# bluecube/minipath

Hardware: AMD Instinct MI355X
Metric: Mrays/s (higher is better)
Workload: dtype f32; 1 GPU; atrium stand-in for the absent data/Sponza (reference .gitmodules:1-3: un-fetched submodule), 258432 triangles, generator seed 1; 1920x1080 256spp tile64 seed0x5eed depth1 (reference semantics: primary ray + |d.n|, worker.rs:51-66); parallelism=tiles round-robin over 1 rank(s)

## Files before the change

### minipath_amd/csrc/kernels.hip

```cpp
#include <hip/hip_runtime.h>

#include <algorithm>
#include <cfloat>
#include <cmath>
#include <cstdlib>
#include <type_traits>

#include "launch_plan.h"
#include "mp_internal.h"
#include "family_launch.h"
#include "ray_math.h"

#ifdef MP_PROF_MISSES
namespace mp {
namespace {
__device__ unsigned long long g_prof[8];
}
}
#define MP_PROF_COUNT(i) do { if ((threadIdx.x & 63u) == 0u) atomicAdd(&g_prof[i], 1ull); } while (0)
#endif
#include "mask_cache.h"
#include "group_walk.h"

namespace mp {
// ... 327 lines not shown
                const float hx = fms(r.dy, e2z, r.dz * e2y), hy = fms(r.dz, e2x, r.dx * e2z), hz = fms(r.dx, e2y, r.dy * e2x);
                const float det = fma_dot(e1x, e1y, e1z, hx, hy, hz);
                const float sx = r.ox - v0x, sy = r.oy - v0y, sz = r.oz - v0z;
                const float un = fma_dot(sx, sy, sz, hx, hy, hz);
                const uint32_t det_sign = as_u(det) & 0x80000000u;
                const bool det_ok = fabsf(det) <= kHuge;
                const float xu = det_ok ? as_f(as_u(un) ^ det_sign) : 1.0f;
                if (__ballot(!(xu <= thr)) == 0) return;
                const float qx = fms(sy, e1z, sz * e1y), qy = fms(sz, e1x, sx * e1z), qz = fms(sx, e1y, sy * e1x);
                const float vn = fma_dot(r.dx, r.dy, r.dz, qx, qy, qz);
                const float tn = fma_dot(e2x, e2y, e2z, qx, qy, qz);
                const float xv = det_ok ? as_f(as_u(vn) ^ det_sign) : 1.0f, xt = det_ok ? as_f(as_u(tn) ^ det_sign) : 1.0f;
                if (__ballot(!(fminf(fminf(xu, xv), xt) <= thr)) == 0) return;
                const float inv_det = 1.0f / det;
                const float u = inv_det * un, v = inv_det * vn, t = inv_det * tn;
                const bool acc = (u >= 0.0f) & (v >= 0.0f) & ((u + v) <= 1.0f) & (t >= 0.0f) & (t < lim);
                best_t = acc ? t : best_t;
                lim = acc ? t : lim;
                bu = acc ? u : bu;
                bv = acc ? v : bv;
                bprim = acc ? tri : bprim;
                changed |= __ballot(acc);
            };
            float a0 = tp[0], a1 = tp[1], a2 = tp[2], a3 = tp[3], a4 = tp[4], a5 = tp[5], a6 = tp[6], a7 = tp[7], a8 = tp[8];
            uint32_t tri = first * 8u;
            for (uint32_t p = n_real >> 1; p > 0; p--) {
                const float b0 = tp[9], b1 = tp[10], b2 = tp[11], b3 = tp[12], b4 = tp[13], b5 = tp[14], b6 = tp[15], b7 = tp[16], b8 = tp[17];
                test(a0, a1, a2, a3, a4, a5, a6, a7, a8, tri);
                a0 = tp[18]; a1 = tp[19]; a2 = tp[20]; a3 = tp[21]; a4 = tp[22]; a5 = tp[23]; a6 = tp[24]; a7 = tp[25]; a8 = tp[26];
                test(b0, b1, b2, b3, b4, b5, b6, b7, b8, tri + 1u);
                tri += 2u;
                tp += 2 * kTriDwords;
            }
            if (n_real & 1u) test(a0, a1, a2, a3, a4, a5, a6, a7, a8, tri);
            if (changed != 0) stale_top = sp;
        }
    }
    hit.t = best_t; hit.u = bu; hit.v = bv; hit.prim = bprim;
}

struct RegStack3 {
    int ent, mlo, mhi;
    __device__ __forceinline__ RegStack3() : ent(0), mlo(0), mhi(0) {}
    __device__ __forceinline__ void push(int sp, uint32_t e, uint64_t m) {
        asm volatile("s_mov_b32 m0, %3\n\ts_nop 0\n\t"
                     "v_writelane_b32 %0, %4, m0\n\tv_writelane_b32 %1, %5, m0\n\tv_writelane_b32 %2, %6, m0"
                     : "+v"(ent), "+v"(mlo), "+v"(mhi)
                     : "s"(sp), "s"(e), "s"(static_cast<uint32_t>(m)), "s"(static_cast<uint32_t>(m >> 32))
                     : "m0");
    }
    __device__ __forceinline__ void pop(int sp, uint32_t& e, uint64_t& m) const {
        e = static_cast<uint32_t>(__builtin_amdgcn_readlane(ent, sp));
        m = static_cast<uint32_t>(__builtin_amdgcn_readlane(mlo, sp)) |
            (static_cast<uint64_t>(static_cast<uint32_t>(__builtin_amdgcn_readlane(mhi, sp))) << 32);
    }
};

template <int OCT>
__device__ __noinline__ uint32_t unit_list_slow(const float* __restrict__ nodes_pk, uint32_t* mcache, uint32_t node, uint32_t slots) {
    return unit_list_build(reinterpret_cast<const float4*>(nodes_pk), mcache, node, slots,
                           [](const float* b, const float bmn[3], const float bmx[3]) { return bounds_may_hit<OCT>(b, bmn, bmx); });
}
template <int OCT>
__device__ __forceinline__ bool trace_packet_cached(const DevScene& sc, const Ray& r, bool active, PacketHit& hit, uint32_t* mcache) {
    static_assert(kNullLink == MP_LINK_NULL, "mask_cache.h's copy of the null link");
    kfp nodes = (kfp)(uintptr_t)sc.nodes_pk;
    kfp tris = (kfp)(uintptr_t)sc.tris_aos;
    float best_t = FLT_MAX, bu = 0.0f, bv = 0.0f;
    uint32_t bprim = kNoPrim;
    RegStack3 st;
    int sp = 0;
    mcache[kRootListSlot] = sc.pk_count * sc.pk_mask_bits;
    wave_lds_sync();
    uint32_t cur = (static_cast<uint32_t>(kRootListSlot) << 16) | 1u;
    uint64_t pm = __ballot(active);
    for (;;) {
        if ((cur & 0xFFFFu) == 0u) {
            if (sp == 0) break;
            sp--;
            st.pop(sp, cur, pm);
        }
        cur -= 1u;
        const uint32_t src = __builtin_amdgcn_readfirstlane(mcache[(cur >> 16) + (cur & 0xFFFFu)]);
        const bool pon = __builtin_amdgcn_inverse_ballot_w64(pm);
        const krec8 rec = *reinterpret_cast<const __attribute__((address_space(4))) krec8*>(reinterpret_cast<const __attribute__((address_space(4))) char*>(nodes) + scalar_u(src * 32u));
        float t1, t2;
        slab<false, OCT>(rec[0], rec[1], rec[2], rec[3], rec[4], rec[5], r, pon ? best_t : -1.0f, t1, t2);
        const bool ok = t1 <= t2;
        if (__ballot(ok) == 0) continue;
        const uint32_t link = uniform_u(rec[6]);
        float lim = ok ? best_t : -1.0f;
        if ((link & 63u) == 0u) {
            MP_PROF_COUNT(2);
            const uint32_t node = link >> 6;
            const uint32_t slot = node_slot(node);
            const uint32_t tag = __builtin_amdgcn_readfirstlane(mcache[static_cast<uint32_t>(kMaskCacheHeader) + slot]);
            uint32_t list = __builtin_amdgcn_readfirstlane(mcache[static_cast<uint32_t>(kNodeListBase) + slot]);
            if (__builtin_expect(tag != node, 0)) {
                MP_PROF_COUNT(0);
                if (tag != 0xFFFFFFFFu) MP_PROF_COUNT(4);
                list = __builtin_amdgcn_readfirstlane(unit_list_slow<OCT>(sc.nodes_pk, mcache, node, sc.pk_mask_bits));
                if (list == kListOverflow) {
                    if (sp != 0 || (cur & 0xFFFFu) != 0u) {
                        MP_PROF_COUNT(6);
                        return false;
                    }
                    list = __builtin_amdgcn_readfirstlane(unit_list_slow<OCT>(sc.nodes_pk, mcache, node, sc.pk_mask_bits));
                }
            }
            if ((list & 0xFFFFu) != 0u) {
                if ((cur & 0xFFFFu) != 0u) {
                    st.push(sp, cur, pm);
                    sp++;
                }
                cur = list;
                pm = __ballot(lim >= 0.0f);
            }
        } else {
            const uint32_t first = link >> 6, n_real = link & 63u;
            kfp tp = tris + static_cast<size_t>(first) * (8 * kTriDwords);
            const float thr = lim >= 0.0f ? -kTiny : INFINITY;
            auto test = [&](const float v0x, const float v0y, const float v0z, const float e1x, const float e1y, const float e1z,
                            const float e2x, const float e2y, const float e2z, const uint32_t tri) {
                const float hx = fms(r.dy, e2z, r.dz * e2y), hy = fms(r.dz, e2x, r.dx * e2z), hz = fms(r.dx, e2y, r.dy * e2x);
                const float det = fma_dot(e1x, e1y, e1z, hx, hy, hz);
                const float sx = r.ox - v0x, sy = r.oy - v0y, sz = r.oz - v0z;
                const float un = fma_dot(sx, sy, sz, hx, hy, hz);
                const uint32_t det_sign = as_u(det) & 0x80000000u;
                const bool det_ok = fabsf(det) <= kHuge;
                const float xu = det_ok ? as_f(as_u(un) ^ det_sign) : 1.0f;
                if (__ballot(!(xu <= thr)) == 0) return;
                const float qx = fms(sy, e1z, sz * e1y), qy = fms(sz, e1x, sx * e1z), qz = fms(sx, e1y, sy * e1x);
                const float vn = fma_dot(r.dx, r.dy, r.dz, qx, qy, qz);
                const float tn = fma_dot(e2x, e2y, e2z, qx, qy, qz);
                const float xv = det_ok ? as_f(as_u(vn) ^ det_sign) : 1.0f, xt = det_ok ? as_f(as_u(tn) ^ det_sign) : 1.0f;
                if (__ballot(!(fminf(fminf(xu, xv), xt) <= thr)) == 0) return;
                constexpr uint32_t kRcpLo = 0x10800000u , kRcpHi = 0x7E000000u ;
                const uint32_t wkey = (as_u(det) << 1) - (kRcpLo << 1);
                const float inv_det = __ballot(wkey > ((kRcpHi - kRcpLo) << 1)) == 0 ? rm::rcp_short(det) : 1.0f / det;
                const float u = inv_det * un, v = inv_det * vn, t = inv_det * tn;
                const bool acc = !(fminf(fminf(u, v), t) < 0.0f) & ((u + v) <= 1.0f) & (t < lim);
                best_t = acc ? t : best_t;
                lim = acc ? t : lim;
                bu = acc ? u : bu;
                bv = acc ? v : bv;
                bprim = acc ? tri : bprim;
            };
            const uint32_t ls = first & static_cast<uint32_t>(kLeafCacheEntries - 1);
            const uint32_t tag = mcache[kLeafTagBase + ls];
            const uint2 tm = reinterpret_cast<const uint2*>(mcache + kLeafMaskBase)[ls];
            uint64_t todo;
            if (__builtin_expect(__builtin_amdgcn_readfirstlane(tag) == first, 1)) {
                todo = __builtin_amdgcn_readfirstlane(tm.x) | (static_cast<uint64_t>(__builtin_amdgcn_readfirstlane(tm.y)) << 32);
            } else {
                MP_PROF_COUNT(1);
                const uint64_t m = leaf_mask_slow(sc.tris_aos, mcache, first, n_real);
                todo = __builtin_amdgcn_readfirstlane(static_cast<uint32_t>(m)) | (static_cast<uint64_t>(__builtin_amdgcn_readfirstlane(static_cast<uint32_t>(m >> 32))) << 32);
            }
            if (todo != 0) {
                uint32_t c = static_cast<uint32_t>(__builtin_ctzll(todo));
                todo &= ~(1ull << c);
                kfp ta = tri_record(tp, c);
                krec8 ra = *reinterpret_cast<const __attribute__((address_space(4))) krec8*>(ta);
                float a8 = ta[8];
                while (todo != 0) {
                    const uint32_t cn = static_cast<uint32_t>(__builtin_ctzll(todo));
                    todo &= ~(1ull << cn);
                    kfp tb = tri_record(tp, cn);
                    const krec8 rb = *reinterpret_cast<const __attribute__((address_space(4))) krec8*>(tb);
                    const float b8 = tb[8];
                    test(ra[0], ra[1], ra[2], ra[3], ra[4], ra[5], ra[6], ra[7], a8, first * 8u + c);
                    ra = rb; a8 = b8;
                    c = cn;
                }
                test(ra[0], ra[1], ra[2], ra[3], ra[4], ra[5], ra[6], ra[7], a8, first * 8u + c);
            }
        }
    }
    hit.t = best_t; hit.u = bu; hit.v = bv; hit.prim = bprim;
    return true;
}

template <bool OCTANTS, class Stack, bool MC = false>
__device__ __forceinline__ void trace_packet(const DevScene& sc, const Ray& r, bool active, Stack& st, PacketHit& hit,
                                             const MaskCache& mc = MaskCache{nullptr}) {
    if (OCTANTS && MC) {
        if (__ballot(active & !mask_cache_ray_ok(r)) != 0) {
            const bool slow = active && (fabsf(r.ix) == INFINITY || fabsf(r.iy) == INFINITY || fabsf(r.iz) == INFINITY);
            if (__ballot(slow) != 0) trace_packet_impl<2, -1>(sc, r, active, st, hit);
            else trace_packet_impl<1, -1>(sc, r, active, st, hit);
            return;
        }
    } else {
        const bool slow = active && (fabsf(r.ix) == INFINITY || fabsf(r.iy) == INFINITY || fabsf(r.iz) == INFINITY);
        if (__ballot(slow) != 0) {
            trace_packet_impl<2, -1>(sc, r, active, st, hit);
            return;
        }
    }
    if (OCTANTS && sc.boxes_ordered) {
        const uint64_t am = __ballot(active);
        const uint64_t nx = __ballot(active && r.ix < 0.0f), ny = __ballot(active && r.iy < 0.0f), nz = __ballot(active && r.iz < 0.0f);
        if ((nx == 0 || nx == am) && (ny == 0 || ny == am) && (nz == 0 || nz == am)) {
            const uint32_t oct = (nx ? 1u : 0u) | (ny ? 2u : 0u) | (nz ? 4u : 0u);
            if (MC) {
                mask_cache_begin_pass(mc, r, active, oct);
                bool done;
                switch (oct) {
                    case 0: done = trace_packet_cached<0>(sc, r, active, hit, mc.lds); break;
                    case 1: done = trace_packet_cached<1>(sc, r, active, hit, mc.lds); break;
                    case 2: done = trace_packet_cached<2>(sc, r, active, hit, mc.lds); break;
                    case 3: done = trace_packet_cached<3>(sc, r, active, hit, mc.lds); break;
                    case 4: done = trace_packet_cached<4>(sc, r, active, hit, mc.lds); break;
                    case 5: done = trace_packet_cached<5>(sc, r, active, hit, mc.lds); break;
                    case 6: done = trace_packet_cached<6>(sc, r, active, hit, mc.lds); break;
                    default: done = trace_packet_cached<7>(sc, r, active, hit, mc.lds); break;
                }
                if (done) return;
            } else {
                switch (oct) {
                    case 0: trace_packet_impl<1, 0>(sc, r, active, st, hit); return;
                    case 1: trace_packet_impl<1, 1>(sc, r, active, st, hit); return;
                    case 2: trace_packet_impl<1, 2>(sc, r, active, st, hit); return;
                    case 3: trace_packet_impl<1, 3>(sc, r, active, st, hit); return;
                    case 4: trace_packet_impl<1, 4>(sc, r, active, st, hit); return;
                    case 5: trace_packet_impl<1, 5>(sc, r, active, st, hit); return;
                    case 6: trace_packet_impl<1, 6>(sc, r, active, st, hit); return;
                    default: trace_packet_impl<1, 7>(sc, r, active, st, hit); return;
                }
            }
        }
    }
    trace_packet_impl<1, -1>(sc, r, active, st, hit);
}

template <class T>
__device__ __forceinline__ const T* uniform_ptr(const T* p) {
    const uint64_t v = reinterpret_cast<uint64_t>(p);
    const uint32_t lo = __builtin_amdgcn_readfirstlane(static_cast<uint32_t>(v)), hi = __builtin_amdgcn_readfirstlane(static_cast<uint32_t>(v >> 32));
    return reinterpret_cast<const T*>((static_cast<uint64_t>(hi) << 32) | lo);
}
// ... 1549 lines not shown
```

### minipath_amd/csrc/mask_cache.h

```cpp
#pragma once

#include <hip/hip_runtime.h>

#include <cfloat>
#include <cmath>
#include <cstdint>

#include "camera_rays.h"

#ifndef MP_PROF_COUNT
#define MP_PROF_COUNT(i) do { } while (0)
#endif

namespace mp {
namespace mc {
__device__ __forceinline__ float as_f(uint32_t u) { return __uint_as_float(u); }
__device__ __forceinline__ uint32_t as_u(float f) { return __float_as_uint(f); }

__device__ __forceinline__ void wave_lds_sync() {
    __builtin_amdgcn_fence(__ATOMIC_RELEASE, "wavefront");
    __builtin_amdgcn_wave_barrier();
    __builtin_amdgcn_fence(__ATOMIC_ACQUIRE, "wavefront");
}

// ... 148 lines not shown
            for (int g = 0; g < 3; g++) {
#pragma unroll
                for (int k = 0; k < 3; k++) { hdr[hdr_lo(g) + k] = pmin[g][k]; hdr[hdr_lo(g) + 3 + k] = pmax[g][k]; }
            }
            mc.lds[kHdrState] = oct | 0x100u;
        }
        int l_ = lane;
        asm volatile("" : "+v"(l_));
#pragma unroll
        for (int i = 0; i < (kMaskCacheEntries + kLeafCacheEntries) / 64; i++) mc.lds[kMaskCacheHeader + i * 64 + l_] = 0xFFFFFFFFu;
        wave_lds_sync();
    }
}
#ifndef MP_MCACHE_MARGIN
#define MP_MCACHE_MARGIN 0.015625f
#endif
__device__ __forceinline__ void mask_cache_begin_unit(const MaskCache& mc, const mp_camera_sampler& s, float jitter_scale, uint32_t x0,
                                                      uint32_t x1, uint32_t y0, uint32_t y1) {
    const int lane = static_cast<int>(threadIdx.x) & 63;
    Ray r;
    float f[3];
    camera_film(s, (lane & 1) ? static_cast<float>(x1) + (jitter_scale + (-0.5f)) : static_cast<float>(x0) + (-0.5f),
                (lane & 2) ? static_cast<float>(y1) + (jitter_scale + (-0.5f)) : static_cast<float>(y0) + (-0.5f), f);
    camera_lens_ray(s, f, (lane & 4) ? 1.0f : -1.0f, (lane & 8) ? 1.0f : -1.0f, r);
    const uint64_t nx = __ballot(r.ix < 0.0f), ny = __ballot(r.iy < 0.0f), nz = __ballot(r.iz < 0.0f);
    const bool adopt = __ballot(!mask_cache_ray_ok(r)) == 0 && (nx == 0 || ~nx == 0) && (ny == 0 || ~ny == 0) && (nz == 0 || ~nz == 0);
    if (!adopt) {
        if (lane == 0) mc.lds[kHdrState] = 0xFFFFFFFFu;
        wave_lds_sync();
        return;
    }
    const uint32_t oct = (nx ? 1u : 0u) | (ny ? 2u : 0u) | (nz ? 4u : 0u);
    float pmin[3][3] = {{r.ox, r.oy, r.oz}, {r.ix, r.iy, r.iz}, {r.dx, r.dy, r.dz}}, pmax[3][3];
#pragma unroll
    for (int g = 0; g < 3; g++) {
#pragma unroll
        for (int k = 0; k < 3; k++) pmax[g][k] = pmin[g][k];
        wave_min3_max3(pmin[g], pmax[g]);
    }
    float* hdr = reinterpret_cast<float*>(mc.lds);
    if (lane == 63) {
#pragma unroll
        for (int g = 0; g < 3; g++) {
#pragma unroll
            for (int k = 0; k < 3; k++) {
                const float lo = pmin[g][k], hi = pmax[g][k];
                const float pad = (hi - lo) * MP_MCACHE_MARGIN;
                float wlo = lo - pad, whi = hi + pad;
                if (g == 1) {
                    if ((wlo < 0.0f) != (lo < 0.0f) || wlo == 0.0f) wlo = lo;
                    if ((whi < 0.0f) != (hi < 0.0f) || whi == 0.0f) whi = hi;
                    if (!(fabsf(wlo) < INFINITY)) wlo = lo;
                    if (!(fabsf(whi) < INFINITY)) whi = hi;
                } else {
                    const float cap = g == 0 ? 2.0f * kCoordCap : 2.0f;
                    wlo = fmaxf(wlo, -cap); whi = fminf(whi, cap);
                }
                hdr[hdr_lo(g) + k] = wlo; hdr[hdr_lo(g) + 3 + k] = whi;
            }
        }
        mc.lds[kHdrState] = oct | 0x100u;
    }
    MP_PROF_COUNT(3);
#pragma unroll
    for (int i = 0; i < (kMaskCacheEntries + kLeafCacheEntries) / 64; i++) mc.lds[kMaskCacheHeader + i * 64 + lane] = 0xFFFFFFFFu;
    wave_lds_sync();
}
template <int OCT>
__device__ __forceinline__ bool bounds_may_hit(const float* b, const float bmn[3], const float bmx[3]) {
    float L[3], U[3];
#pragma unroll
    for (int k = 0; k < 3; k++) {
        const float y = bmn[k] - b[3 + k], z = bmx[k] - b[k];
        const float lo_src = ((OCT >> k) & 1) ? z : y, hi_src = ((OCT >> k) & 1) ? y : z;
        L[k] = fminf(lo_src * b[6 + k], lo_src * b[9 + k]);
        U[k] = fmaxf(hi_src * b[6 + k], hi_src * b[9 + k]);
    }
    const float t1 = fmaxf(fmaxf(L[0], 0.0f), fmaxf(L[1], L[2])), t2 = fminf(U[0], fminf(U[1], U[2]));
    return !(t1 > t2);
}

constexpr uint32_t kNullLink = 0xFFFFFFF8u;
constexpr uint32_t kListOverflow = 0xFFFFFFFFu;
constexpr int kListDepth = 64;
__device__ __forceinline__ uint32_t node_slot(uint32_t node) {
    return min(node & static_cast<uint32_t>(kMaskCacheEntries - 1) & MP_NODE_SLOT_MASK, static_cast<uint32_t>(kMaskCacheEntries - 2));
}
template <class Kept>
__device__ __forceinline__ uint32_t unit_list_build(const float4* __restrict__ recs, uint32_t* mcache, uint32_t node, uint32_t slots, Kept kept) {
    const uint32_t lane = threadIdx.x & 63u;
    const float* b = reinterpret_cast<const float*>(mcache);
    node = __builtin_amdgcn_readfirstlane(node);
    slots = __builtin_amdgcn_readfirstlane(slots);
    auto kept_of = [&](uint32_t n, float4& c0, float4& c1) -> uint32_t {
        bool keep = false;
        c0 = make_float4(0.0f, 0.0f, 0.0f, 0.0f); c1 = c0;
        if (lane < slots) {
            const float4* r = recs + (static_cast<size_t>(n) * slots + lane) * 2;
            c0 = r[0]; c1 = r[1];
            const float bmn[3] = {c0.x, c0.y, c0.z}, bmx[3] = {c0.w, c1.x, c1.y};
            keep = as_u(c1.z) != kNullLink && kept(b, bmn, bmx);
        }
        return __builtin_amdgcn_readfirstlane(static_cast<uint32_t>(__ballot(keep)));
    };
    float4 c0, c1;
    uint32_t mask = kept_of(node, c0, c1);
    const uint32_t top = ~__builtin_amdgcn_readfirstlane(mcache[kArenaTopSlot]);
    if (top > static_cast<uint32_t>(kArenaEntries) || top + static_cast<uint32_t>(__popc(mask)) > static_cast<uint32_t>(kArenaEntries)) {
        MP_PROF_COUNT(5);
        wave_lds_sync();
#pragma unroll
        for (int i = 0; i < (kMaskCacheEntries + 63) / 64; i++)
            if (i * 64 + static_cast<int>(lane) < kMaskCacheEntries) mcache[kMaskCacheHeader + i * 64 + static_cast<int>(lane)] = 0xFFFFFFFFu;
        wave_lds_sync();
        return kListOverflow;
    }
    const uint32_t room = static_cast<uint32_t>(kArenaEntries) - top;
    uint32_t used = 0u, pend = static_cast<uint32_t>(__popc(mask)), cur = node;
    int st_node = 0, st_mask = 0, depth = 0;
    for (;;) {
        if (mask == 0u) {
            while (mask == 0u && depth > 0) {
                depth--;
                cur = static_cast<uint32_t>(__builtin_amdgcn_readlane(st_node, depth));
                mask = static_cast<uint32_t>(__builtin_amdgcn_readlane(st_mask, depth));
            }
            if (mask == 0u) break;
            if (lane < slots) {
                const float4* r = recs + (static_cast<size_t>(cur) * slots + lane) * 2;
                c0 = r[0]; c1 = r[1];
            }
        }
        const uint32_t j = static_cast<uint32_t>(__builtin_ctz(mask));
        mask &= mask - 1u;
        pend--;
        const uint32_t rec = cur * slots + j;
        auto from_lane = [&](float v) { return as_f(static_cast<uint32_t>(__builtin_amdgcn_readlane(static_cast<int>(as_u(v)), static_cast<int>(j)))); };
        const float4 p0 = make_float4(from_lane(c0.x), from_lane(c0.y), from_lane(c0.z), from_lane(c0.w));
        const float4 p1 = make_float4(from_lane(c1.x), from_lane(c1.y), from_lane(c1.z), 0.0f);
        const uint32_t link = as_u(p1.z);
        bool emit = true;
        if ((link & 63u) == 0u) {
            const uint32_t m = link >> 6;
            float4 g0, g1;
            const uint32_t km = kept_of(m, g0, g1);
            const bool sticks_out = ((km >> lane) & 1u) != 0u && lane < slots &&
                                    !(p0.x <= g0.x && p0.y <= g0.y && p0.z <= g0.z && g0.w <= p0.w && g1.x <= p1.x && g1.y <= p1.y);
            if (km == 0u) {
                emit = false;
            } else if (__ballot(sticks_out) == 0 && depth < kListDepth && used + pend + static_cast<uint32_t>(__popc(km)) <= room) {
                if (mask != 0u) {
                    asm volatile("s_mov_b32 m0, %2\n\ts_nop 0\n\tv_writelane_b32 %0, %3, m0\n\tv_writelane_b32 %1, %4, m0"
                                 : "+v"(st_node), "+v"(st_mask) : "s"(depth), "s"(__builtin_amdgcn_readfirstlane(cur)), "s"(__builtin_amdgcn_readfirstlane(mask)) : "m0");
                    depth++;
                }
                cur = m; mask = km; pend += static_cast<uint32_t>(__popc(km));
                c0 = g0; c1 = g1;
                emit = false;
            }
        }
        if (emit) {
            if (lane == 0u) mcache[static_cast<uint32_t>(kArenaBase) + top + used] = rec;
            used++;
        }
    }
    const uint32_t val = ((static_cast<uint32_t>(kArenaBase) + top) << 16) | used;
    if (lane == 0u) {
        const uint32_t slot = node_slot(node);
        mcache[static_cast<uint32_t>(kMaskCacheHeader) + slot] = node;
        mcache[static_cast<uint32_t>(kNodeListBase) + slot] = val;
        mcache[kArenaTopSlot] = ~(top + used);
    }
    wave_lds_sync();
    return val;
}

struct Iv {
    float lo, hi;
};
__device__ __forceinline__ Iv iv_neg(const Iv a) { return Iv{-a.hi, -a.lo}; }
__device__ __forceinline__ Iv iv_mul_c(const Iv a, const float c) {
    const float p = a.lo * c, q = a.hi * c;
    return Iv{fminf(p, q), fmaxf(p, q)};
}
__device__ __forceinline__ Iv iv_mul(const Iv a, const Iv b) {
    const float p1 = a.lo * b.lo, p2 = a.lo * b.hi, p3 = a.hi * b.lo, p4 = a.hi * b.hi;
    return Iv{fminf(fminf(p1, p2), fminf(p3, p4)), fmaxf(fmaxf(p1, p2), fmaxf(p3, p4))};
}
__device__ __forceinline__ Iv iv_fma_c(const Iv a, const float c, const Iv z) {
    return Iv{fminf(__builtin_fmaf(a.lo, c, z.lo), __builtin_fmaf(a.hi, c, z.lo)), fmaxf(__builtin_fmaf(a.lo, c, z.hi), __builtin_fmaf(a.hi, c, z.hi))};
}
__device__ __forceinline__ Iv iv_fma(const Iv a, const Iv b, const Iv z) {
    const float l1 = __builtin_fmaf(a.lo, b.lo, z.lo), l2 = __builtin_fmaf(a.lo, b.hi, z.lo), l3 = __builtin_fmaf(a.hi, b.lo, z.lo), l4 = __builtin_fmaf(a.hi, b.hi, z.lo);
    const float h1 = __builtin_fmaf(a.lo, b.lo, z.hi), h2 = __builtin_fmaf(a.lo, b.hi, z.hi), h3 = __builtin_fmaf(a.hi, b.lo, z.hi), h4 = __builtin_fmaf(a.hi, b.hi, z.hi);
    return Iv{fminf(fminf(l1, l2), fminf(l3, l4)), fmaxf(fmaxf(h1, h2), fmaxf(h3, h4))};
}
__device__ __forceinline__ bool tri_may_hit(const float* b, const float (&v0)[3], const float (&e1)[3], const float (&e2)[3]) {
    const Iv d[3] = {Iv{b[13], b[16]}, Iv{b[14], b[17]}, Iv{b[15], b[18]}};
    const Iv h[3] = {iv_fma_c(d[1], e2[2], iv_neg(iv_mul_c(d[2], e2[1]))), iv_fma_c(d[2], e2[0], iv_neg(iv_mul_c(d[0], e2[2]))),
                     iv_fma_c(d[0], e2[1], iv_neg(iv_mul_c(d[1], e2[0])))};
    const Iv det = iv_fma_c(h[2], e1[2], iv_fma_c(h[1], e1[1], iv_mul_c(h[0], e1[0])));
    if (!(det.lo > 0.0f || det.hi < 0.0f)) return true;
    const Iv inv = Iv{1.0f / det.hi, 1.0f / det.lo};
    if (!(fabsf(inv.lo) < INFINITY && fabsf(inv.hi) < INFINITY)) return true;
    const Iv s[3] = {Iv{b[0] - v0[0], b[3] - v0[0]}, Iv{b[1] - v0[1], b[4] - v0[1]}, Iv{b[2] - v0[2], b[5] - v0[2]}};
    const Iv u = iv_mul(inv, iv_fma(s[2], h[2], iv_fma(s[1], h[1], iv_mul(s[0], h[0]))));
    const Iv q[3] = {iv_fma_c(s[1], e1[2], iv_neg(iv_mul_c(s[2], e1[1]))), iv_fma_c(s[2], e1[0], iv_neg(iv_mul_c(s[0], e1[2]))),
                     iv_fma_c(s[0], e1[1], iv_neg(iv_mul_c(s[1], e1[0])))};
    const Iv v = iv_mul(inv, iv_fma(d[2], q[2], iv_fma(d[1], q[1], iv_mul(d[0], q[0]))));
    const Iv t = iv_mul(inv, iv_fma_c(q[2], e2[2], iv_fma_c(q[1], e2[1], iv_mul_c(q[0], e2[0]))));
    const bool miss = u.hi < 0.0f || v.hi < 0.0f || (u.lo + v.lo) > 1.0f || t.hi < 0.0f;
    return !miss;
}

}
}
```

### minipath_amd/csrc/mask_probe.hip

```cpp
#include <hip/hip_runtime.h>

#include <cfloat>
#include <cstdint>

#include "mask_cache.h"

namespace {

using namespace mp::mc;

constexpr int kCounters = 8;
constexpr float kOrgCap = 2.0f * kCoordCap;

__device__ __forceinline__ uint64_t mix64(uint64_t z) {
    z = (z ^ (z >> 30)) * 0xbf58476d1ce4e5b9ull;
    z = (z ^ (z >> 27)) * 0x94d049bb133111ebull;
    return z ^ (z >> 31);
}
__device__ __forceinline__ uint64_t hsh(uint64_t seed, uint64_t c, uint32_t k) { return mix64(seed ^ mix64(c * 0x10000ull + k)); }
__device__ __forceinline__ float unit(uint64_t h) { return static_cast<float>(static_cast<uint32_t>(h >> 40)) * 0x1p-24f; }

__device__ __forceinline__ void record_case(unsigned long long* out, bool bad, uint64_t idx, bool hit, bool rejected, bool edge_only) {
    if ((threadIdx.x & 63) != 0) return;
    atomicAdd(out + 1, 1ull);
// ... 121 lines not shown
        if (mode == 2u) {
            const uint64_t hn = hsh(seed, c, 42);
            const uint32_t n = 1u + static_cast<uint32_t>(hn & 3u), kk = static_cast<uint32_t>(hn >> 8) % 3u, which = static_cast<uint32_t>(hn >> 16) & 3u;
            const bool up = (hn >> 24) & 1u;
            for (uint32_t i = 0; i < n; i++) {
#pragma unroll
                for (int k = 0; k < 3; k++) {
                    if (static_cast<uint32_t>(k) != kk) continue;
                    if (which == 0u || which == 3u) v0[k] = step(v0[k], up);
                    if (which == 1u || which == 3u) v1[k] = step(v1[k], up);
                    if (which == 2u || which == 3u) v2[k] = step(v2[k], up);
                }
            }
        }
    } else if (mode == 3u) {
        const uint32_t sub = static_cast<uint32_t>(hm >> 20) & 3u, ax = static_cast<uint32_t>(hm >> 24) % 3u;
#pragma unroll
        for (int k = 0; k < 3; k++) {
            v0[k] = p[k];
            if (sub == 0u) { v1[k] = k == static_cast<int>(ax) ? p[k] + E1[k] : p[k]; v2[k] = k == static_cast<int>(ax) ? p[k] - E2[k] : p[k]; }
            else if (sub == 1u) { v1[k] = p[k]; v2[k] = p[k] + E2[k]; }
            else if (sub == 2u) { v1[k] = p[k] + E1[k]; v2[k] = v1[k]; }
            else { v1[k] = p[k] + E1[k]; v2[k] = p[k] + 2.0f * E1[k]; }
        }
    } else if (mode == 4u) {
        const uint32_t ax = static_cast<uint32_t>(hm >> 20) % 3u;
        const float f = clampf((hm >> 24) & 1u ? b[3 + ax] : b[ax], -kCoordCap, kCoordCap);
        const float a = unit(hsh(seed, c, 40)), bb = unit(hsh(seed, c, 41)) * (1.0f - a);
#pragma unroll
        for (int k = 0; k < 3; k++) {
            v0[k] = p[k] - a * E1[k] - bb * E2[k];
            v1[k] = v0[k] + E1[k];
            v2[k] = v0[k] + E2[k];
            if (k == static_cast<int>(ax)) v0[k] = v1[k] = v2[k] = f;
        }
    } else {
#pragma unroll
        for (int k = 0; k < 3; k++) {
            const float ctr = 0.5f * b[k] + 0.5f * b[3 + k];
            v0[k] = ctr + pick(hsh(seed, c, 50 + k), 127 - 30, 127 + 30);
            v1[k] = ctr + pick(hsh(seed, c, 53 + k), 127 - 30, 127 + 30);
            v2[k] = ctr + pick(hsh(seed, c, 56 + k), 127 - 30, 127 + 30);
        }
    }
    clamp_vertex(v0); clamp_vertex(v1); clamp_vertex(v2);
}

constexpr int kDumpHead = 40, kDumpRay = 10, kRays = 192;
constexpr int kDumpCase = kDumpHead + kRays * kDumpRay;

__global__ void tri_kernel(uint64_t seed, uint64_t base, uint64_t ncases, unsigned long long* out, uint32_t* dump) {
    const uint64_t c = base + (static_cast<uint64_t>(blockIdx.x) * blockDim.x + threadIdx.x) / 64u;
    const uint32_t lane = threadIdx.x & 63u;
    if (c >= ncases) return;
    float b[20], v0[3], v1[3], v2[3];
    gen_tri_case(seed, c, b, v0, v1, v2);
    const float e1[3] = {v1[0] - v0[0], v1[1] - v0[1], v1[2] - v0[2]}, e2[3] = {v2[0] - v0[0], v2[1] - v0[1], v2[2] - v0[2]};
    float lo[6], hi[6];
#pragma unroll
    for (int k = 0; k < 3; k++) { lo[k] = b[k]; hi[k] = b[3 + k]; lo[3 + k] = b[13 + k]; hi[3 + k] = b[16 + k]; }
    const bool keep = tri_may_hit(b, v0, e1, e2);
    bool edge = false, inner = false;
    uint32_t* rec = dump ? dump + c * kDumpCase : nullptr;
    for (uint32_t s = 0; s < 3; s++) {
        const uint32_t j = s * 64u + lane;
        float x[6];
        case_ray(lo, hi, j, seed, c, x);
        const TriRay tr = mt_ray(x, v0, e1, e2);
        if (s < 2) edge |= tr.hit; else inner |= tr.hit;
        if (rec) {
            uint32_t* rr = rec + kDumpHead + j * kDumpRay;
            for (int k = 0; k < 6; k++) rr[k] = as_u(x[k]);
            rr[6] = as_u(tr.t); rr[7] = as_u(tr.u); rr[8] = as_u(tr.v); rr[9] = tr.hit ? 1u : 0u;
        }
    }
    const bool any_edge = __ballot(edge) != 0, any_inner = __ballot(inner) != 0, any = any_edge || any_inner;
    if (rec && lane < 20u) rec[lane] = as_u(b[lane]);
    if (rec && lane == 20u) {
        for (int k = 0; k < 3; k++) { rec[20 + k] = as_u(v0[k]); rec[23 + k] = as_u(v1[k]); rec[26 + k] = as_u(v2[k]); }
        for (int k = 0; k < 3; k++) { rec[29 + k] = as_u(e1[k]); rec[32 + k] = as_u(e2[k]); }
        rec[35] = keep ? 1u : 0u;
    }
    record_case(out, !keep && any, c, any, !keep, any_edge && !any_inner);
}

__device__ __forceinline__ void gen_box_case(uint64_t seed, uint64_t c, uint32_t oct, float (&b)[20], float (&bmn)[3], float (&bmx)[3]) {
    float olo[3], ohi[3];
    gen_origin_bounds(seed, c, olo, ohi);
#pragma unroll
    for (int k = 0; k < 3; k++) {
        const uint64_t h = hsh(seed, c, 60 + k), h2 = hsh(seed, c, 63 + k);
        const bool wide = (h & 0x300u) == 0u;
        float m1 = wide ? pick_pos(h, 1, 254) : pick_pos(h, 127 - 2, 127 + 12);
        float m2 = (h2 & 7u) == 0u ? m1 : wide ? pick_pos(h2, 1, 254) : pick_pos(h2, 127 - 2, 127 + 12);
        if ((h2 & 0x7F00u) == 0u) m2 = FLT_MAX;
        const float mlo = fminf(m1, m2), mhi = fmaxf(m1, m2);
        const bool neg = ((oct >> k) & 1u) != 0u;
        b[k] = olo[k]; b[3 + k] = ohi[k];
        b[6 + k] = neg ? -mhi : mlo;
        b[9 + k] = neg ? -mlo : mhi;
    }
    b[12] = as_f(oct | 0x100u);
    for (int i = 13; i < 20; i++) b[i] = 0.0f;
    float lo[6], hi[6];
#pragma unroll
    for (int k = 0; k < 3; k++) { lo[k] = b[k]; hi[k] = b[3 + k]; lo[3 + k] = b[6 + k]; hi[3 + k] = b[9 + k]; }
    const uint64_t hm = hsh(seed, c, 70);
    const uint32_t mode = static_cast<uint32_t>(hm & 7u);
    float x[6];
    const uint32_t j = (hm & 0x300u) ? static_cast<uint32_t>(hm >> 10) & 127u : 128u + (static_cast<uint32_t>(hm >> 10) & 63u);
    case_ray(lo, hi, j, seed, c, x);
    const float d[3] = {1.0f / x[3], 1.0f / x[4], 1.0f / x[5]};
    const uint64_t ht = hsh(seed, c, 71);
    const float t = mode == 2u ? -pick_pos(ht, 127 - 10, 127 + 30) : (ht & 3u) == 0u ? 0.0f : pick_pos(ht, 127 - 30, 127 + 30);
    float half[3];
#pragma unroll
    for (int k = 0; k < 3; k++) {
        const float p = x[k] + t * d[k];
        half[k] = pick_pos(hsh(seed, c, 72 + k), 127 - 30, 127 + 31);
        bmn[k] = p - half[k];
        bmx[k] = p + half[k];
    }
    if (mode == 0u) {
        const uint32_t m = 1u + static_cast<uint32_t>(hm >> 20) % 7u;
#pragma unroll
        for (int k = 0; k < 3; k++) if ((m >> k) & 1u) bmx[k] = bmn[k] = (hm >> (24 + k)) & 1u ? x[k] + t * d[k] : bmn[k];
    } else if (mode == 1u) {
#pragma unroll
        for (int k = 0; k < 3; k++) {
            const uint32_t f = static_cast<uint32_t>(hm >> (20 + 3 * k)) & 7u;
            if (f == 1u) bmn[k] = b[k]; else if (f == 2u) bmn[k] = b[3 + k]; else if (f == 3u) bmx[k] = b[k]; else if (f == 4u) bmx[k] = b[3 + k];
            else if (f == 5u) { bmn[k] = b[k]; bmx[k] = b[3 + k]; }
            if (bmn[k] > bmx[k]) { const float s = bmn[k]; bmn[k] = bmx[k]; bmx[k] = s; }
        }
    } else if (mode == 3u) {
#pragma unroll
        for (int k = 0; k < 3; k++) {
            const uint32_t f = static_cast<uint32_t>(hm >> (20 + 2 * k)) & 3u;
            bmn[k] = f == 1u ? x[k] : x[k] - half[k];
            bmx[k] = f == 2u ? x[k] : x[k] + half[k];
        }
    } else if (mode == 4u) {
        const uint32_t a = static_cast<uint32_t>(hm >> 20) % 3u, e = (a + 1u + (static_cast<uint32_t>(hm >> 24) & 1u)) % 3u, o3 = 3u - a - e;
        const float T = pick_pos(ht, 127 - 20, 127 + 20), big = 0x1p40f;
        float xa = x[a] + T * d[a];
        const float Ta = (xa - x[a]) * x[3 + a];
        float ye = x[e] + Ta * d[e];
        for (int i = -4; i <= 4; i++) {
            float y = ye;
            for (int s = 0; s < (i < 0 ? -i : i); s++) y = step(y, i > 0);
            if ((y - x[e]) * x[3 + e] == Ta) { ye = y; break; }
        }
        const bool na = x[3 + a] < 0.0f, ne = x[3 + e] < 0.0f;
        bmn[a] = na ? xa - big : xa; bmx[a] = na ? xa : xa + big;
        bmn[e] = ne ? ye : ye - big; bmx[e] = ne ? ye + big : ye;
        bmn[o3] = x[o3] - big; bmx[o3] = x[o3] + big;
    } else if (mode == 5u) {
#pragma unroll
        for (int k = 0; k < 3; k++) {
            const uint32_t f = static_cast<uint32_t>(hm >> (20 + 2 * k)) & 3u;
            if (f == 1u) bmn[k] = -FLT_MAX; else if (f == 2u) bmx[k] = FLT_MAX; else if (f == 3u) { bmn[k] = -FLT_MAX; bmx[k] = FLT_MAX; }
        }
    }
#pragma unroll
    for (int k = 0; k < 3; k++) {
        bmn[k] = clampf(bmn[k], -FLT_MAX, FLT_MAX); bmx[k] = clampf(bmx[k], -FLT_MAX, FLT_MAX);
// ... 268 lines not shown
                           [](const float* b, const float bmn[3], const float bmx[3]) { return bounds_may_hit<OCT>(b, bmn, bmx); });
}
__global__ void __launch_bounds__(256) list_kernel(const float4* recs, uint32_t slots, const uint32_t* headers, const uint32_t* cases, uint32_t n,
                                                   uint32_t* out) {
    __shared__ __align__(16) uint32_t lds[4 * kMaskCacheDwords];
    const uint32_t w = threadIdx.x >> 6, lane = threadIdx.x & 63u;
    const uint32_t c = blockIdx.x * 4u + w;
    if (c >= n) return;
    uint32_t* const base = lds + w * kMaskCacheDwords;
    for (uint32_t i = lane; i < static_cast<uint32_t>(kMaskCacheDwords); i += 64u)
        base[i] = i < static_cast<uint32_t>(kMaskCacheHeader) ? headers[32u * c + i] : i < static_cast<uint32_t>(kLeafMaskBase) ? 0xFFFFFFFFu : 0xDEAD0000u + i;
    wave_lds_sync();
    const uint32_t node = cases[2u * c], top0 = cases[2u * c + 1u];
    if (lane == 0u) base[kArenaTopSlot] = ~top0;
    wave_lds_sync();
    uint32_t val;
    switch (__builtin_amdgcn_readfirstlane(base[kHdrState]) & 7u) {
        case 0: val = list_slow<0>(recs, base, node, slots); break;
        case 1: val = list_slow<1>(recs, base, node, slots); break;
        case 2: val = list_slow<2>(recs, base, node, slots); break;
        case 3: val = list_slow<3>(recs, base, node, slots); break;
        case 4: val = list_slow<4>(recs, base, node, slots); break;
        case 5: val = list_slow<5>(recs, base, node, slots); break;
        case 6: val = list_slow<6>(recs, base, node, slots); break;
        default: val = list_slow<7>(recs, base, node, slots); break;
    }
    wave_lds_sync();
    uint32_t* const o = out + static_cast<size_t>(c) * kListOut;
    if (lane == 0u) {
        const uint32_t slot = node_slot(node);
        o[0] = val; o[1] = ~base[kArenaTopSlot]; o[2] = base[static_cast<uint32_t>(kMaskCacheHeader) + slot]; o[3] = base[static_cast<uint32_t>(kNodeListBase) + slot];
    }
    for (uint32_t i = lane; i < static_cast<uint32_t>(kArenaRoom); i += 64u) o[4u + i] = base[static_cast<uint32_t>(kArenaBase) + i];
}

template <class F>
int run(F launch, unsigned long long* host) {
    (void)hipGetLastError();
    unsigned long long* dev = nullptr;
    unsigned long long init[kCounters] = {0ull, 0ull, ~0ull, 0ull, 0ull, 0ull, 0ull, 0ull};
    hipError_t e = hipMalloc(&dev, sizeof(init));
    if (e != hipSuccess) return static_cast<int>(e);
    e = hipMemcpy(dev, init, sizeof(init), hipMemcpyHostToDevice);
    if (e == hipSuccess) {
        launch(dev);
        e = hipGetLastError();
        if (e == hipSuccess) e = hipDeviceSynchronize();
        if (e == hipSuccess) e = hipMemcpy(host, dev, sizeof(init), hipMemcpyDeviceToHost);
    }
    const hipError_t ef = hipFree(dev);
    return static_cast<int>(e != hipSuccess ? e : ef);
}
void merge(unsigned long long* acc, const unsigned long long* r) {
    for (int i = 0; i < kCounters; i++) if (i != 2) acc[i] += r[i];
    if (r[2] < acc[2]) acc[2] = r[2];
}
void reset(unsigned long long* acc) {
    for (int i = 0; i < kCounters; i++) acc[i] = 0ull;
    acc[2] = ~0ull;
}
constexpr uint64_t kCasesPerLaunch = 1ull << 20;

template <class K>
int run_cases(K kernel, uint64_t seed, uint64_t ncases, uint32_t* dump_dev, unsigned long long* out) {
    unsigned long long acc[kCounters];
    reset(acc);
    for (uint64_t c0 = 0; c0 < ncases; c0 += kCasesPerLaunch) {
        const uint64_t n = ncases - c0 < kCasesPerLaunch ? ncases - c0 : kCasesPerLaunch;
        unsigned long long r[kCounters];
        if (int rc = run([&](unsigned long long* d) {
                hipLaunchKernelGGL(kernel, dim3(static_cast<uint32_t>((n + 3) / 4)), dim3(256), 0, 0, seed, c0, c0 + n, d, dump_dev);
            }, r))
            return rc;
        merge(acc, r);
    }
    for (int i = 0; i < kCounters; i++) out[i] = acc[i];
    return 0;
}

}

extern "C" {
int mp_mask_probe_tri(uint64_t seed, uint64_t ncases, unsigned long long* out) { return run_cases(tri_kernel, seed, ncases, nullptr, out); }
int mp_mask_probe_box(uint64_t seed, uint64_t ncases, unsigned long long* out) { return run_cases(box_kernel, seed, ncases, nullptr, out); }
int mp_mask_probe_dump_dwords() { return kDumpCase; }
int mp_mask_probe_dump(int kind, uint64_t seed, uint64_t ncases, uint32_t* host, unsigned long long* out) {
    (void)hipGetLastError();
    uint32_t* dev = nullptr;
    const size_t bytes = static_cast<size_t>(ncases) * kDumpCase * sizeof(uint32_t);
    hipError_t e = hipMalloc(&dev, bytes);
    if (e != hipSuccess) return static_cast<int>(e);
    e = hipMemset(dev, 0, bytes);
    int rc = static_cast<int>(e);
    if (e == hipSuccess) rc = kind == 0 ? run_cases(tri_kernel, seed, ncases, dev, out) : run_cases(box_kernel, seed, ncases, dev, out);
    if (rc == 0) rc = static_cast<int>(hipMemcpy(host, dev, bytes, hipMemcpyDeviceToHost));
    const hipError_t ef = hipFree(dev);
    return rc != 0 ? rc : static_cast<int>(ef);
}
int mp_mask_probe_ray_ok(uint64_t seed, unsigned long long* out) {
    unsigned long long acc[kCounters];
    reset(acc);
    constexpr uint64_t kThreads = (1ull << 32) / kOkPerThread, kBlocks = kThreads / 256;
    for (int comp = 0; comp < 9; comp++) {
        unsigned long long r[kCounters];
        if (int rc = run([&](unsigned long long* d) {
                hipLaunchKernelGGL(ray_ok_kernel, dim3(static_cast<uint32_t>(kBlocks)), dim3(256), 0, 0, seed, comp, 0ull, d);
            }, r))
            return rc;
        if (r[2] != ~0ull) r[2] += static_cast<unsigned long long>(comp) << 32;
        merge(acc, r);
    }
    for (int i = 0; i < kCounters; i++) out[i] = acc[i];
    return 0;
}
int mp_mask_probe_dev(uint64_t seed, const float* set, uint32_t n, uint64_t nrandom, unsigned long long* out) {
    (void)hipGetLastError();
    float* dset = nullptr;
    hipError_t e = hipMalloc(&dset, sizeof(float) * (n ? n : 1u));
    if (e != hipSuccess) return static_cast<int>(e);
    e = hipMemcpy(dset, set, sizeof(float) * n, hipMemcpyHostToDevice);
    int rc = static_cast<int>(e);
    unsigned long long acc[kCounters];
    reset(acc);
    const uint64_t ntrip = static_cast<uint64_t>(n) * n * n;
    if (rc == 0 && ntrip) {
        unsigned long long r[kCounters];
        rc = run([&](unsigned long long* d) {
            hipLaunchKernelGGL(dev_kernel, dim3(static_cast<uint32_t>((ntrip + 255) / 256)), dim3(256), 0, 0, seed, 0, 0ull, n, dset, d);
        }, r);
        if (rc == 0) merge(acc, r);
    }
    if (rc == 0 && nrandom) {
        unsigned long long r[kCounters];
        rc = run([&](unsigned long long* d) {
            hipLaunchKernelGGL(dev_kernel, dim3(static_cast<uint32_t>((nrandom + 255) / 256)), dim3(256), 0, 0, seed, 1, 0ull, n, dset, d);
        }, r);
        if (rc == 0) { if (r[2] != ~0ull) r[2] += 1ull << 40; merge(acc, r); }
    }
    const hipError_t ef = hipFree(dset);
    if (rc != 0) return rc;
    for (int i = 0; i < kCounters; i++) out[i] = acc[i];
    return static_cast<int>(ef);
}
int mp_mask_probe_unit(const float* sampler, float jitter_scale, const uint32_t* blocks, uint32_t n, uint32_t* out, uint32_t* ntags,
                       float* margin) {
    (void)hipGetLastError();
    *ntags = static_cast<uint32_t>(kLeafMaskBase - kMaskCacheHeader);
    *margin = MP_MCACHE_MARGIN;
    if (n == 0u) return 0;
    SamplerArg cam;
    const float* p = sampler;
    for (int k = 0; k < 3; k++) { cam.s.center[k] = p[k]; cam.s.up[k] = p[3 + k]; cam.s.right[k] = p[6 + k]; cam.s.film_origin_offset[k] = p[9 + k]; }
    cam.s.pixel_scale = p[12]; cam.s.lens_radius = p[13]; cam.s.lens_weight = p[14];
    uint32_t *dblocks = nullptr, *dout = nullptr;
    hipError_t e = hipMalloc(&dblocks, sizeof(uint32_t) * 4u * n);
    if (e == hipSuccess) e = hipMalloc(&dout, sizeof(uint32_t) * kUnitOut * n);
    if (e == hipSuccess) e = hipMemcpy(dblocks, blocks, sizeof(uint32_t) * 4u * n, hipMemcpyHostToDevice);
    if (e == hipSuccess) {
        hipLaunchKernelGGL(unit_kernel, dim3((n + 3u) / 4u), dim3(256), 0, 0, cam, jitter_scale, dblocks, n, dout);
        e = hipGetLastError();
        if (e == hipSuccess) e = hipDeviceSynchronize();
        if (e == hipSuccess) e = hipMemcpy(out, dout, sizeof(uint32_t) * kUnitOut * n, hipMemcpyDeviceToHost);
    }
    (void)hipFree(dblocks);
    (void)hipFree(dout);
    return static_cast<int>(e);
// ... 39 lines not shown
```

Baseline: 35990 Mrays/s.

## Skip cached empty leaves and add far-side early exit to triangle test

When a leaf's cached triangle mask comes out empty, the traversal now marks that list entry in LDS with a high bit, so later visits skip the node fetch and slab test. The triangle test also gains a far-side early exit: it leaves the wave early when barycentrics exceed |det|, not only when they are negative. A probe kernel is added to count how often the new exits fire. The LDS write plus wave sync on the empty path adds some cost, and the wider exit condition carries a small risk of wrongly culling near-edge hits.

```diff
diff --git a/minipath_amd/csrc/kernels.hip b/minipath_amd/csrc/kernels.hip
--- a/minipath_amd/csrc/kernels.hip
+++ b/minipath_amd/csrc/kernels.hip
@@ -433,6 +433,12 @@
         }
         cur -= 1u;
         const uint32_t src = __builtin_amdgcn_readfirstlane(mcache[(cur >> 16) + (cur & 0xFFFFu)]);
+#ifndef MP_NO_EMPTY_SKIP
+        if (static_cast<int32_t>(src) < 0) {
+            MP_PROF_COUNT(7);
+            continue;
+        }
+#endif
         const bool pon = __builtin_amdgcn_inverse_ballot_w64(pm);
         const krec8 rec = *reinterpret_cast<const __attribute__((address_space(4))) krec8*>(reinterpret_cast<const __attribute__((address_space(4))) char*>(nodes) + scalar_u(src * 32u));
         float t1, t2;
@@ -470,6 +476,7 @@
         } else {
             const uint32_t first = link >> 6, n_real = link & 63u;
             kfp tp = tris + static_cast<size_t>(first) * (8 * kTriDwords);
+            static_assert(kExitTiny == kTiny && kExitHuge == kHuge, "mask_cache.h's copies of the early-out constants");
             const float thr = lim >= 0.0f ? -kTiny : INFINITY;
             auto test = [&](const float v0x, const float v0y, const float v0z, const float e1x, const float e1y, const float e1z,
                             const float e2x, const float e2y, const float e2z, const uint32_t tri) {
@@ -477,15 +484,13 @@
                 const float det = fma_dot(e1x, e1y, e1z, hx, hy, hz);
                 const float sx = r.ox - v0x, sy = r.oy - v0y, sz = r.oz - v0z;
                 const float un = fma_dot(sx, sy, sz, hx, hy, hz);
-                const uint32_t det_sign = as_u(det) & 0x80000000u;
-                const bool det_ok = fabsf(det) <= kHuge;
-                const float xu = det_ok ? as_f(as_u(un) ^ det_sign) : 1.0f;
-                if (__ballot(!(xu <= thr)) == 0) return;
+                const float xu = tri_flipped(det, un);
+                if (__ballot(!(tri_exit1_key(det, xu) <= thr)) == 0) return;
                 const float qx = fms(sy, e1z, sz * e1y), qy = fms(sz, e1x, sx * e1z), qz = fms(sx, e1y, sy * e1x);
                 const float vn = fma_dot(r.dx, r.dy, r.dz, qx, qy, qz);
                 const float tn = fma_dot(e2x, e2y, e2z, qx, qy, qz);
-                const float xv = det_ok ? as_f(as_u(vn) ^ det_sign) : 1.0f, xt = det_ok ? as_f(as_u(tn) ^ det_sign) : 1.0f;
-                if (__ballot(!(fminf(fminf(xu, xv), xt) <= thr)) == 0) return;
+                const float xv = tri_flipped(det, vn), xt = tri_flipped(det, tn);
+                if (__ballot(!(tri_exit2_key(det, xu, xv, xt) <= thr)) == 0) return;
                 constexpr uint32_t kRcpLo = 0x10800000u , kRcpHi = 0x7E000000u ;
                 const uint32_t wkey = (as_u(det) << 1) - (kRcpLo << 1);
                 const float inv_det = __ballot(wkey > ((kRcpHi - kRcpLo) << 1)) == 0 ? rm::rcp_short(det) : 1.0f / det;
@@ -508,6 +513,12 @@
                 const uint64_t m = leaf_mask_slow(sc.tris_aos, mcache, first, n_real);
                 todo = __builtin_amdgcn_readfirstlane(static_cast<uint32_t>(m)) | (static_cast<uint64_t>(__builtin_amdgcn_readfirstlane(static_cast<uint32_t>(m >> 32))) << 32);
             }
+#ifndef MP_NO_EMPTY_SKIP
+            if (todo == 0 && (cur >> 16) != static_cast<uint32_t>(kRootListSlot)) {
+                if ((threadIdx.x & 63u) == 0u) mcache[(cur >> 16) + (cur & 0xFFFFu)] = src | kEmptyLeafBit;
+                wave_lds_sync();
+            }
+#endif
             if (todo != 0) {
                 uint32_t c = static_cast<uint32_t>(__builtin_ctzll(todo));
                 todo &= ~(1ull << c);
diff --git a/minipath_amd/csrc/mask_cache.h b/minipath_amd/csrc/mask_cache.h
--- a/minipath_amd/csrc/mask_cache.h
+++ b/minipath_amd/csrc/mask_cache.h
@@ -254,6 +254,7 @@
 
 constexpr uint32_t kNullLink = 0xFFFFFFF8u;
 constexpr uint32_t kListOverflow = 0xFFFFFFFFu;
+constexpr uint32_t kEmptyLeafBit = 0x80000000u;
 constexpr int kListDepth = 64;
 __device__ __forceinline__ uint32_t node_slot(uint32_t node) {
     return min(node & static_cast<uint32_t>(kMaskCacheEntries - 1) & MP_NODE_SLOT_MASK, static_cast<uint32_t>(kMaskCacheEntries - 2));
@@ -385,5 +386,28 @@
     return !miss;
 }
 
-}
-}
+constexpr float kExitTiny = 9.094947017729282e-13f;
+constexpr float kExitHuge = 1099511627776.0f;
+constexpr float kFarSlack = 1.00000095367431640625f;
+__device__ __forceinline__ float tri_flipped(float det, float num) {
+    return fabsf(det) <= kExitHuge ? as_f(as_u(num) ^ (as_u(det) & 0x80000000u)) : 1.0f;
+}
+__device__ __forceinline__ float tri_far_key(float det, float x) { return __builtin_fmaf(fabsf(det), kFarSlack, -x); }
+__device__ __forceinline__ float tri_exit1_key(float det, float xu) {
+#ifdef MP_NO_FAR_EXIT
+    return xu;
+#else
+    return fminf(xu, tri_far_key(det, xu));
+#endif
+}
+__device__ __forceinline__ float tri_exit2_key(float det, float xu, float xv, float xt) {
+    const float near_key = fminf(fminf(xu, xv), xt);
+#ifdef MP_NO_FAR_EXIT
+    return near_key;
+#else
+    return fminf(fminf(near_key, tri_far_key(det, xu)), tri_far_key(det, xu + xv));
+#endif
+}
+
+}
+}
diff --git a/minipath_amd/csrc/mask_probe.hip b/minipath_amd/csrc/mask_probe.hip
--- a/minipath_amd/csrc/mask_probe.hip
+++ b/minipath_amd/csrc/mask_probe.hip
@@ -227,6 +227,42 @@
         rec[35] = keep ? 1u : 0u;
     }
     record_case(out, !keep && any, c, any, !keep, any_edge && !any_inner);
+}
+
+__global__ void exit_kernel(uint64_t seed, uint64_t base, uint64_t ncases, unsigned long long* out, uint32_t*) {
+    const uint64_t c = base + (static_cast<uint64_t>(blockIdx.x) * blockDim.x + threadIdx.x) / 64u;
+    const uint32_t lane = threadIdx.x & 63u;
+    if (c >= ncases) return;
+    float b[20], v0[3], v1[3], v2[3];
+    gen_tri_case(seed, c, b, v0, v1, v2);
+    const float e1[3] = {v1[0] - v0[0], v1[1] - v0[1], v1[2] - v0[2]}, e2[3] = {v2[0] - v0[0], v2[1] - v0[1], v2[2] - v0[2]};
+    float lo[6], hi[6];
+#pragma unroll
+    for (int k = 0; k < 3; k++) { lo[k] = b[k]; hi[k] = b[3 + k]; lo[3 + k] = b[13 + k]; hi[3 + k] = b[16 + k]; }
+    float x[6];
+    case_ray(lo, hi, static_cast<uint32_t>(c % 3u) * 64u + lane, seed, c, x);
+    const uint64_t hl = hsh(seed, c, 90);
+    const uint64_t live_mask = (hl & 7u) == 0u ? ~0ull : (hsh(seed, c, 91) | (1ull << (hl >> 58)));
+    const bool live = ((live_mask >> lane) & 1u) != 0u;
+    const float dx = x[3], dy = x[4], dz = x[5];
+    const float hx = fms(dy, e2[2], dz * e2[1]), hy = fms(dz, e2[0], dx * e2[2]), hz = fms(dx, e2[1], dy * e2[0]);
+    const float det = fma_dot(e1[0], e1[1], e1[2], hx, hy, hz);
+    const float sx = x[0] - v0[0], sy = x[1] - v0[1], sz = x[2] - v0[2];
+    const float un = fma_dot(sx, sy, sz, hx, hy, hz);
+    const float thr = live ? -kExitTiny : INFINITY;
+    const float xu = tri_flipped(det, un);
+    const bool exit1 = __ballot(!(tri_exit1_key(det, xu) <= thr)) == 0;
+    const float qx = fms(sy, e1[2], sz * e1[1]), qy = fms(sz, e1[0], sx * e1[2]), qz = fms(sx, e1[1], sy * e1[0]);
+    const float vn = fma_dot(dx, dy, dz, qx, qy, qz);
+    const float tn = fma_dot(e2[0], e2[1], e2[2], qx, qy, qz);
+    const float xv = tri_flipped(det, vn), xt = tri_flipped(det, tn);
+    const bool exit2 = __ballot(!(tri_exit2_key(det, xu, xv, xt) <= thr)) == 0;
+    const bool near1 = __ballot(!(xu <= thr)) == 0, near2 = __ballot(!(fminf(fminf(xu, xv), xt) <= thr)) == 0;
+    const TriRay tr = mt_ray(x, v0, e1, e2);
+    const bool any = __ballot(live && tr.hit) != 0;
+    const bool left = exit1 || exit2;
+    record_case(out, left && any, c, any, exit1, exit2 && !exit1);
+    if (lane == 0u && left && !(near1 || near2)) atomicAdd(out + 6, 1ull);
 }
 
 __device__ __forceinline__ void gen_box_case(uint64_t seed, uint64_t c, uint32_t oct, float (&b)[20], float (&bmn)[3], float (&bmx)[3]) {
@@ -661,6 +697,7 @@
 
 extern "C" {
 int mp_mask_probe_tri(uint64_t seed, uint64_t ncases, unsigned long long* out) { return run_cases(tri_kernel, seed, ncases, nullptr, out); }
+int mp_mask_probe_exits(uint64_t seed, uint64_t ncases, unsigned long long* out) { return run_cases(exit_kernel, seed, ncases, nullptr, out); }
 int mp_mask_probe_box(uint64_t seed, uint64_t ncases, unsigned long long* out) { return run_cases(box_kernel, seed, ncases, nullptr, out); }
 int mp_mask_probe_dump_dwords() { return kDumpCase; }
 int mp_mask_probe_dump(int kind, uint64_t seed, uint64_t ncases, uint32_t* host, unsigned long long* out) {
```

Result: faster. 37780 Mrays/s (median of 6 runs) (+5.0%).
